# LBM-EPFL/MaD

Hardware: NVIDIA B200
Metric: voxels/sec scale-space+detect+describe(+match) (higher is better)
Workload: dtype f32 grids, f64 line accumulation, u8 x u8 -> s32 matching

## Files before the change

### include/mad_b200.h

```cpp
#ifndef MAD_B200_H
#define MAD_B200_H

#include <stddef.h>
#include <stdint.h>

#ifdef __cplusplus
extern "C" {
#endif

#define MAD_OK 0
#define MAD_ERR_ARG (-1)
#define MAD_ERR_CUDA (-2)
#define MAD_ERR_CAPACITY (-3)
#define MAD_ERR_NODEVICE (-4)

#define MAD_MAX_ORI 36
#define MAD_DSC_LEN 1024

typedef struct MadKeypoint {
    int32_t vox[3];
    int32_t oct;
    float off[3];
    float val;
    int32_t peak[3];
// ... 21 lines not shown
const char* mad_last_error_string(void);
int mad_version(void);
int mad_device_info(int* sm_count, int* cc_major, int* cc_minor);

int mad_publish_small(const void* src_dev, void* dst_host_mapped, int bytes, void* stream);

int mad_copy_to_host(const void* src_dev, void* dst_host_mapped, long long bytes, int n_ctas, void* stream);

long long mad_launch_count(void);
int mad_profile_enable(int on);
int mad_profile_count(void);
int mad_profile_get(int i, const char** name, float* ms);
int mad_profile_reset(void);

int mad_grid_max(const float* grid, long long n, float* out_max_ord, void* stream);
float mad_grid_max_decode(unsigned int ord);
int mad_threshold_normalise(float* grid, long long n, float isovalue, float vmax, int divide, void* stream);
int mad_grid_bbox(const float* grid, int nx, int ny, int nz, int* bbox6, void* stream);
int mad_crop_pad3d(const float* in, int nx, int ny, int nz, int x0, int y0, int z0, int cx, int cy, int cz,
                   int pad, float* out, void* stream);

int mad_pad3d(const float* in, int nx, int ny, int nz, int pad, float* out, void* stream);

size_t mad_upsample_workspace_bytes(int bx, int by, int bz);
int mad_upsample_presmooth(const float* base, int bx, int by, int bz,
                           const double* gauss_w_host, int radius,
                           float* up, void* workspace, size_t workspace_bytes, void* stream);

size_t mad_log_gauss_workspace_bytes(int nx, int ny, int nz);
int mad_log_gauss(const float* grid, int nx, int ny, int nz,
                  const double* w0_host, const double* w2_host, int radius, float scale,
                  float* log_out, float* gauss_out, void* workspace, size_t workspace_bytes,
                  int exact_f64, void* stream);

int mad_gradient(const float* gauss, int nx, int ny, int nz, float* grad4, void* stream);
size_t mad_gradient_tiles(int nx, int ny, int nz);
int mad_gradient_mark(const MadKeypoint* kp, int n_kp, const int* dims_oct_host, int reach_oct0, int reach_oct1,
                      uint8_t* flags_oct0, uint8_t* flags_oct1, void* stream);
int mad_gradient_masked(const float* gauss, int nx, int ny, int nz, float* grad4, uint8_t* flags, void* stream);

int mad_detect(const float* log_grid, int nx, int ny, int nz, int oct, int border,
               float threshold, MadKeypoint* cand, int cap, int* count, void* stream);

size_t mad_sort_keypoints_workspace_bytes(int n);
int mad_sort_keypoints(const MadKeypoint* cand, int n, const int* dims_oct_host,
                       MadKeypoint* out, int* out_count,
                       void* workspace, size_t workspace_bytes, void* stream);

int mad_orient(const float* grad4_oct0, const float* grad4_oct1, const int* dims_oct_host,
               const MadKeypoint* kp, int n_kp, int r, const MadZoneTable* zones112_host,
               const double* r1_table, int lim_main, int lim_sec,
               int32_t* n_ori, int32_t* slots, void* stream);

size_t mad_compact_oriented_workspace_bytes(int n_kp);
int mad_compact_oriented(const int32_t* n_ori, const int32_t* slots, int n_kp,
                         MadOriented* oriented, int cap, int* out_count,
                         void* workspace, size_t workspace_bytes, void* stream);

int mad_describe(const float* grad4_oct0, const float* grad4_oct1, const int* dims_oct_host,
                 const MadKeypoint* kp, const MadOriented* oriented, int n_oriented, int r,
                 const MadZoneTable* zones16_host, const double* rf_table, const double* rf_inv_table,
                 int rf_zones, int16_t* dsc, void* stream);

typedef struct MadDscSet {
    const int16_t* dsc;
    const void* half;
// ... 70 lines not shown
```

### mad_b200/_lib.py

```python
import ctypes as C
import os

import numpy as np

HERE = os.path.dirname(os.path.abspath(__file__))
LIB_PATH = os.path.join(HERE, "libmad_b200.so")


class MadError(RuntimeError):
    pass


if not os.path.exists(LIB_PATH):
    raise ImportError(
        "mad_b200: %s is missing -- build the CUDA library first (python -m mad_b200.build). "
        "There is no CPU fallback." % LIB_PATH)

lib = C.CDLL(LIB_PATH)

KEYPOINT_DTYPE = np.dtype([("vox", "<i4", 3), ("oct", "<i4"), ("off", "<f4", 3), ("val", "<f4"),
                           ("peak", "<i4", 3), ("accepted", "<i4")])
ORIENTED_DTYPE = np.dtype([("kp", "<i4"), ("main", "<i2"), ("sec", "<i2")])
assert KEYPOINT_DTYPE.itemsize == 48 and ORIENTED_DTYPE.itemsize == 8
MAX_ORI = 36
# ... 8 lines not shown


class MadDscSet(C.Structure):
    _fields_ = [("dsc", C.c_void_p), ("half", C.c_void_p), ("norm2", C.c_void_p), ("u8", C.c_void_p),
                ("rnorm", C.c_void_p), ("rows", C.c_int32), ("rows_padded", C.c_int32), ("max_entry", C.c_int32)]


_P = C.c_void_p
_I = C.c_int
_SZ = C.c_size_t

SIGNATURES = {
    "mad_last_error_string": (C.c_char_p, []),
    "mad_version": (_I, []),
    "mad_device_info": (_I, [C.POINTER(_I), C.POINTER(_I), C.POINTER(_I)]),
    "mad_launch_count": (C.c_longlong, []),
    "mad_profile_enable": (_I, [_I]),
    "mad_profile_count": (_I, []),
    "mad_profile_get": (_I, [_I, C.POINTER(C.c_char_p), C.POINTER(C.c_float)]),
    "mad_profile_reset": (_I, []),
    "mad_publish_small": (_I, [_P, _P, _I, _P]),
    "mad_copy_to_host": (_I, [_P, _P, C.c_longlong, _I, _P]),
    "mad_zone_fast_build": (_I, [C.POINTER(MadZoneTable), _P, _P]),
    "mad_grid_max": (_I, [_P, C.c_longlong, _P, _P]),
    "mad_grid_max_decode": (C.c_float, [C.c_uint]),
    "mad_threshold_normalise": (_I, [_P, C.c_longlong, C.c_float, C.c_float, _I, _P]),
    "mad_grid_bbox": (_I, [_P, _I, _I, _I, _P, _P]),
    "mad_crop_pad3d": (_I, [_P, _I, _I, _I, _I, _I, _I, _I, _I, _I, _I, _P, _P]),
    "mad_pad3d": (_I, [_P, _I, _I, _I, _I, _P, _P]),
    "mad_upsample_workspace_bytes": (_SZ, [_I, _I, _I]),
    "mad_upsample_presmooth": (_I, [_P, _I, _I, _I, _P, _I, _P, _P, _SZ, _P]),
    "mad_log_gauss_workspace_bytes": (_SZ, [_I, _I, _I]),
    "mad_log_gauss": (_I, [_P, _I, _I, _I, _P, _P, _I, C.c_float, _P, _P, _P, _SZ, _I, _P]),
    "mad_gradient": (_I, [_P, _I, _I, _I, _P, _P]),
    "mad_gradient_tiles": (_SZ, [_I, _I, _I]),
    "mad_gradient_mark": (_I, [_P, _I, _P, _I, _I, _P, _P, _P]),
    "mad_gradient_masked": (_I, [_P, _I, _I, _I, _P, _P, _P]),
    "mad_detect": (_I, [_P, _I, _I, _I, _I, _I, C.c_float, _P, _I, _P, _P]),
    "mad_sort_keypoints_workspace_bytes": (_SZ, [_I]),
    "mad_sort_keypoints": (_I, [_P, _I, _P, _P, _P, _P, _SZ, _P]),
    "mad_orient": (_I, [_P, _P, _P, _P, _I, _I, C.POINTER(MadZoneTable), _P, _I, _I, _P, _P, _P]),
    "mad_compact_oriented_workspace_bytes": (_SZ, [_I]),
    "mad_compact_oriented": (_I, [_P, _P, _I, _P, _I, _P, _P, _SZ, _P]),
    "mad_describe": (_I, [_P, _P, _P, _P, _P, _I, _I, C.POINTER(MadZoneTable), _P, _P, _I, _P, _P]),
    "mad_dsc_prepare": (_I, [_P, _I, _I, _P, _P, _P, _P, _P]),
    "mad_match_pairs": (_I, [C.POINTER(MadDscSet), C.POINTER(MadDscSet), C.c_double, _P, _P, C.c_uint64, _P, _P]),
    "mad_match_pairs_finish_workspace_bytes": (_SZ, [C.c_longlong]),
    "mad_match_pairs_finish": (_I, [_P, _P, C.c_longlong, _I, _I, _P, _P, _P, _P, _P, _P, _SZ, _P]),
    "mad_match_pairs_finish_dot": (_I, [_P, _P, C.c_longlong, _I, _I, _P, _P, _P, _P, _SZ, _P]),
    "mad_dsc_norms": (_I, [_P, _I, _P, _P]),
    "mad_dsc_to_half": (_I, [_P, _I, _I, _P, _P]),
    "mad_match_segments": (_I, [_I, _I, _I]),
    "mad_match_count": (_I, [C.POINTER(MadDscSet), C.POINTER(MadDscSet), C.c_double, _I, _P, _I, _P]),
    "mad_match_fill": (_I, [C.POINTER(MadDscSet), C.POINTER(MadDscSet), C.c_double, _I, _P, _P, _P, _P, _I, _P]),
    "mad_exclusive_scan_workspace_bytes": (_SZ, [_I]),
    "mad_exclusive_scan_i32_to_i64": (_I, [_P, _I, _P, _P, _P, _SZ, _P]),
    "mad_match_topk_workspace_bytes": (_SZ, [_I, _I, _I, _I]),
    "mad_match_topk": (_I, [C.POINTER(MadDscSet), C.POINTER(MadDscSet), _I, _I, _P, _P, _P, _SZ, _I, _P]),
    "mad_topk_merge": (_I, [_P, _P, _I, _I, _I, _P, _P, _P]),
    "mad_density_splat": (_I, [_P, _P, _I, _P, C.c_double, _I, _I, _I, _I, _P, _P]),
    "mad_normalise_f64": (_I, [_P, C.c_longlong, _P, _P]),
    "mad_conv_full_f64": (_I, [_P, C.c_longlong, _I, C.c_longlong, _P, _I, _P, _I, _P]),
    "mad_mark_used": (_I, [_P, C.c_longlong, _P, _P]),
    "mad_repeatability": (_I, [_P, _P, _P, C.c_longlong, _P, _P, _P, _P, _P, _P, _I, _P, _I, _P, _P, _P, _P, _P,
                               C.c_double, _P, _P]),
    "mad_box_scores_workspace_bytes": (_SZ, [_I, _I, _I]),
# ... 26 lines not shown
```

### mad_b200/csrc/scale_space.cu

```cuda
#include <stdlib.h>
#include <type_traits>

#include "common.cuh"

__global__ void __launch_bounds__(256)
pad3d_kernel(const float* __restrict__ in, int nx, int ny, int nz, int pad, float* __restrict__ out, int ox, int oy, int oz) {
    const int lane = threadIdx.x & 31;
    const long long rows = (long long)ox * oy;
    for (long long row = (long long)blockIdx.x * 8 + (threadIdx.x >> 5); row < rows; row += (long long)gridDim.x * 8) {
        const int x = (int)(row / oy), y = (int)(row - (long long)x * oy);
        const int sx = x - pad, sy = y - pad;
        float* o = out + row * oz;
        if (sx < 0 || sx >= nx || sy < 0 || sy >= ny) {
            for (int z = lane; z < oz; z += 32) o[z] = 0.f;
        } else {
            const float* src = in + ((long long)sx * ny + sy) * nz - pad;
            for (int z = lane; z < oz; z += 32) o[z] = (z >= pad && z < nz + pad) ? __ldg(src + z) : 0.f;
        }
    }
}

extern "C" int mad_pad3d(const float* in, int nx, int ny, int nz, int pad, float* out, void* stream) {
    MAD_CHECK_ARG(in && out && nx > 0 && ny > 0 && nz > 0 && pad >= 0);
    const int ox = nx + 2 * pad, oy = ny + 2 * pad, oz = nz + 2 * pad;
// ... 556 lines not shown
    }
#pragma unroll
    for (int jj = R; jj >= 1; --jj) {
#pragma unroll
        for (int t = 0; t < T; ++t) {
            const ACC s = win[t + R - jj] + win[t + R + jj];
            a0[t] = fma(s, Wt<ACC>::get(w.w0[jj]), a0[t]);
            a2[t] = fma(s, Wt<ACC>::get(w.w2[jj]), a2[t]);
        }
    }
#pragma unroll
    for (int t = 0; t < T; ++t) { o0[t] = (float)a0[t]; o2[t] = (float)a2[t]; }
}

template <int R, int T, typename ACC>
__device__ __forceinline__ void conv_g_rows(const ACC* win, const ConvW& w, float* o0) {
    ACC a0[T];
#pragma unroll
    for (int t = 0; t < T; ++t) a0[t] = win[t + R] * Wt<ACC>::get(w.w0[0]);
#pragma unroll
    for (int jj = R; jj >= 1; --jj) {
#pragma unroll
        for (int t = 0; t < T; ++t) {
            const ACC s = win[t + R - jj] + win[t + R + jj];
            a0[t] = fma(s, Wt<ACC>::get(w.w0[jj]), a0[t]);
        }
    }
#pragma unroll
    for (int t = 0; t < T; ++t) o0[t] = (float)a0[t];
}

__device__ __forceinline__ void cp_async4(float* smem_dst, const float* gsrc) {
    asm volatile("cp.async.ca.shared.global [%0], [%1], 4;" ::"r"((uint32_t)__cvta_generic_to_shared(smem_dst)), "l"(gsrc) : "memory");
}
__device__ __forceinline__ void cp_async_commit() { asm volatile("cp.async.commit_group;" ::: "memory"); }
template <int N>
__device__ __forceinline__ void cp_async_wait() { asm volatile("cp.async.wait_group %0;" ::"n"(N) : "memory"); }

template <int R, typename ACC, int MODE>
__global__ void __launch_bounds__(128)
log_pass_strided_kernel(const float* __restrict__ in0, const float* __restrict__ in1, float* __restrict__ o0,
                        float* __restrict__ o1, float* __restrict__ o2, int n, long long inner,
                        long long total_lines, int seg_len, ConvW w) {
    constexpr int T = ((2 * R) % 8 == 0) ? 8 : 4, W = T + 2 * R;
    constexpr int NA = MODE == 1 ? 2 : 1;
    constexpr int D = 32, PF = D / T - 1;
    constexpr int G0 = 2 * R / T;
    static_assert((2 * R) % T == 0, "window prologue must be whole groups");
    extern __shared__ float ring[];
    const long long g = blockIdx.x * (long long)blockDim.x + threadIdx.x;
    if (g >= total_lines) return;
    const long long o = g / inner, j = g % inner;
    const long long base = o * (long long)n * inner + j;
    const int a0 = blockIdx.y * seg_len;
    const int a1 = min(n, a0 + seg_len);
    const int q_end = a1 - a0 + 2 * R;
    float* my = ring + threadIdx.x;
    auto issue = [&](int grp) {
        const int q0 = grp * T;
        float* dst0 = my + ((q0 & (D - 1)) * NA) * 128;
        const int p0 = a0 - R + q0;
        if (p0 >= 0 && p0 + T <= n && q0 + T <= q_end) {
            const long long off = base + (long long)p0 * inner;
#pragma unroll
            for (int i = 0; i < T; ++i) {
                cp_async4(dst0 + i * NA * 128, in0 + off + (long long)i * inner);
// ... 11 lines not shown
            }
        }
        cp_async_commit();
    };
    static_assert(G0 <= PF + 1, "the initial window must fit the ring");
#pragma unroll
    for (int grp = 0; grp <= PF; ++grp) issue(grp);
    cp_async_wait<PF + 1 - G0>();
    ACC wa[W];
    ACC wb[MODE == 1 ? W : 1];
#pragma unroll
    for (int i = 0; i < 2 * R; ++i) {
        wa[i] = (ACC)my[(i * NA) * 128];
        if (MODE == 1) wb[i] = (ACC)my[(i * NA + 1) * 128];
    }
#pragma unroll
    for (int grp = PF + 1; grp <= PF + G0; ++grp) issue(grp);
    int grp = G0;
    for (int a = a0; a < a1; a += T, ++grp) {
        cp_async_wait<PF>();
#pragma unroll
        for (int i = 0; i < T; ++i) {
            const int slot = (grp * T + i) & (D - 1);
            wa[2 * R + i] = (ACC)my[(slot * NA) * 128];
            if (MODE == 1) wb[2 * R + i] = (ACC)my[(slot * NA + 1) * 128];
        }
        issue(grp + PF + 1);
#pragma unroll
        for (int t = 0; t < T; ++t) {
            if (a + t < a1) {
                const long long off = base + (long long)(a + t) * inner;
                float r0, r2;
                conv_both<R, ACC>(wa, t, w, r0, r2);
                o0[off] = r0;
                o1[off] = r2;
                if (MODE == 1) o2[off] = conv_g<R, ACC>(wb, t, w);
            }
        }
#pragma unroll
        for (int i = 0; i < 2 * R; ++i) {
            wa[i] = wa[i + T];
            if (MODE == 1) wb[i] = wb[i + T];
        }
    }
    cp_async_wait<0>();
}

template <int R, typename ACC>
__global__ void __launch_bounds__(384)
log_pass_z_kernel(const float* __restrict__ P01, const float* __restrict__ Rr, const float* __restrict__ S,
                  float* __restrict__ log_out, float* __restrict__ gauss_out, int nz, long long n_rows,
                  int rows_per_cta, int rs_in, int rs_out, long long n_batches, float scale, ConvW w) {
    constexpr int T = 8, W = T + 2 * R;
    extern __shared__ __align__(16) float zsm[];
    const size_t in_buf = (size_t)3 * rows_per_cta * rs_in;
    float* sout0 = zsm + 2 * in_buf;
    float* sout1 = sout0 + (size_t)rows_per_cta * rs_out;
    const int tid = threadIdx.x;
    const int halo_len = nz + 2 * R;
    auto issue = [&](long long batch, int buf) {
        if (batch < n_batches) {
            const long long row0 = batch * rows_per_cta;
            const int rows = (int)min((long long)rows_per_cta, n_rows - row0);
            float* d0 = zsm + buf * in_buf;
            for (int r = 0; r < rows; ++r) {
                const long long gb = (row0 + r) * nz;
                for (int t = tid; t < halo_len; t += blockDim.x) {
                    const long long src = gb + mad_reflect(t - R, nz);
// ... 48 lines not shown
                if (z0 + t < nz) {
                    sout0[r * rs_out + z0 + t] = m;
                    sout1[r * rs_out + z0 + t] = gs[t];
                }
            }
        }
        __syncthreads();
        for (int r = 0; r < rows; ++r) {
            const long long gb = (row0 + r) * nz;
            for (int t = tid; t < nz; t += blockDim.x) {
                log_out[gb + t] = sout0[r * rs_out + t];
                gauss_out[gb + t] = sout1[r * rs_out + t];
            }
        }
    }
    cp_async_wait<0>();
}

template <int R, int DEPTH = 32>
struct YzCfg {
    static constexpr int T = 8, W = T + 2 * R, D = DEPTH, PF = D / T - 1, G0 = 2 * R / T;
    static constexpr int TZ = 128 - 2 * R;
    static constexpr int CH = 128 / T;
    static constexpr int CW = TZ / CH;
    static constexpr int RS = 128;
    static constexpr int OS = TZ;
    static constexpr size_t ring_bytes = (size_t)D * 2 * 128 * sizeof(float);
    static constexpr size_t stage_bytes = (size_t)3 * T * RS * sizeof(double);
    static constexpr size_t out_bytes = (size_t)2 * T * OS * sizeof(float);
    static constexpr size_t smem = ring_bytes + stage_bytes + out_bytes;
    static constexpr bool ok = TZ % CH == 0 && (CW % 2) == 1 && (2 * R) % T == 0 && G0 <= PF + 1;
};

template <int R, typename ACC, int MINB, int DEPTH>
__global__ void __launch_bounds__(128, MINB)
log_pass_yz_kernel(const float* __restrict__ P0, const float* __restrict__ Q0, float* __restrict__ log_out,
                   float* __restrict__ gauss_out, int ny, int nz, int n_ztiles, float scale, ConvW w) {
    using C = YzCfg<R, DEPTH>;
    static_assert(C::ok, "the fused pass needs a kernel radius that is a multiple of 4");
    constexpr int T = C::T, W = C::W, D = C::D, PF = C::PF, G0 = C::G0, TZ = C::TZ, CH = C::CH, CW = C::CW, RS = C::RS, OS = C::OS;
    constexpr int WB = CW + 2 * R;
    extern __shared__ __align__(16) unsigned char yz_smem[];
    float* ring = reinterpret_cast<float*>(yz_smem);
    double* stage = reinterpret_cast<double*>(yz_smem + C::ring_bytes);
    float* sout = reinterpret_cast<float*>(yz_smem + C::ring_bytes + C::stage_bytes);
    const int tid = threadIdx.x;
    const int x = blockIdx.x / n_ztiles, zt = blockIdx.x - x * n_ztiles;
    const int z0 = zt * TZ;
    int zc = z0 - R + tid;
    if (zc >= nz + R) zc = nz + R - 1;
    zc = mad_reflect(zc, nz);
    const long long plane = (long long)x * ny * nz;
    const long long base = plane + zc;
    const int q_end = ny + 2 * R;
    float* my = ring + tid;
    auto issue = [&](int grp) {
        const int q0 = grp * T;
        float* dst0 = my + ((q0 & (D - 1)) * 2) * 128;
        if (q0 >= R && q0 + T <= ny + R) {
            const float* p0 = P0 + base + (long long)(q0 - R) * nz;
            const float* p1 = Q0 + base + (long long)(q0 - R) * nz;
#pragma unroll
            for (int i = 0; i < T; ++i) {
                cp_async4(dst0 + i * 256, p0 + (long long)i * nz);
                cp_async4(dst0 + i * 256 + 128, p1 + (long long)i * nz);
            }
        } else {
#pragma unroll
            for (int i = 0; i < T; ++i) {
                const int q = q0 + i;
                if (q < q_end) {
                    const long long off = base + (long long)mad_reflect(q - R, ny) * nz;
                    cp_async4(dst0 + i * 256, P0 + off);
                    cp_async4(dst0 + i * 256 + 128, Q0 + off);
                }
            }
        }
        cp_async_commit();
    };
#pragma unroll
    for (int grp = 0; grp <= PF; ++grp) issue(grp);
    cp_async_wait<PF + 1 - G0>();
    ACC wa[W], wb[W];
#pragma unroll
    for (int i = 0; i < 2 * R; ++i) {
        wa[i] = (ACC)my[(i * 2) * 128];
        wb[i] = (ACC)my[(i * 2 + 1) * 128];
    }
#pragma unroll
    for (int grp = PF + 1; grp <= PF + G0; ++grp) issue(grp);
    const int br = tid / CH, bc = tid - br * CH;
    const bool b_active = (z0 + bc * CW) < nz;
    int grp = G0;
    for (int a = 0; a < ny; a += T, ++grp) {
        cp_async_wait<PF>();
#pragma unroll
        for (int i = 0; i < T; ++i) {
            const int slot = (grp * T + i) & (D - 1);
            wa[2 * R + i] = (ACC)my[(slot * 2) * 128];
            wb[2 * R + i] = (ACC)my[(slot * 2 + 1) * 128];
        }
        issue(grp + PF + 1);
        {
            float r0[T], r2[T], r1[T];
            conv_both_rows<R, T, ACC>(wa, w, r0, r2);
            conv_g_rows<R, T, ACC>(wb, w, r1);
#pragma unroll
            for (int t = 0; t < T; ++t) {
                const int slot = t * RS + tid;
                stage[0 * T * RS + slot] = (double)r0[t];
                stage[1 * T * RS + slot] = (double)r2[t];
                stage[2 * T * RS + slot] = (double)r1[t];
            }
        }
#pragma unroll
        for (int i = 0; i < 2 * R; ++i) {
            wa[i] = wa[i + T];
            wb[i] = wb[i + T];
        }
        __syncthreads();
        const int rows = min(T, ny - a);
        if (b_active && br < rows) {
            ACC win[WB];
            auto load_window = [&](int arr) {
                const double* src = stage + (arr * T + br) * RS + bc * CW;
#pragma unroll
                for (int q = 0; q < WB; ++q) win[q] = (ACC)src[q];
            };
            float gs[CW], t3[CW], t2[CW], t1[CW];
            load_window(0);
            conv_both_rows<R, CW, ACC>(win, w, gs, t3);
            load_window(1);
            conv_g_rows<R, CW, ACC>(win, w, t2);
            load_window(2);
            conv_g_rows<R, CW, ACC>(win, w, t1);
#pragma unroll
            for (int t = 0; t < CW; ++t) {
                const float lap = __fadd_rn(__fadd_rn(t1[t], t2[t]), t3[t]);
                float m = __fmul_rn(-lap, scale);
                if (m < 0.f) m = 0.f;
                sout[(0 * T + br) * OS + bc * CW + t] = m;
                sout[(1 * T + br) * OS + bc * CW + t] = gs[t];
            }
        }
        __syncthreads();
        if (tid < TZ && z0 + tid < nz) {
            const float* so = sout + tid;
            float* lo_p = log_out + plane + (long long)a * nz + z0 + tid;
            float* ga_p = gauss_out + plane + (long long)a * nz + z0 + tid;
#pragma unroll
            for (int r = 0; r < T; ++r) {
                if (r < rows) {
                    lo_p[(long long)r * nz] = so[(0 * T + r) * OS];
                    ga_p[(long long)r * nz] = so[(1 * T + r) * OS];
                }
            }
        }
    }
    cp_async_wait<0>();
}

extern "C" size_t mad_log_gauss_workspace_bytes(int nx, int ny, int nz) {
    const size_t v = mad_align_up((size_t)nx * ny * nz * sizeof(float), 256);
    return 5 * v;
}

template <int R, typename ACC>
static int log_gauss_launch(const float* grid, int nx, int ny, int nz, const ConvW& w, float scale, float* log_out,
                            float* gauss_out, float* ws, cudaStream_t st) {
    const size_t v = mad_align_up((size_t)nx * ny * nz * sizeof(float), 256) / sizeof(float);
    float *P0 = ws, *Q0 = ws + v, *P01 = ws + 2 * v, *Rr = ws + 3 * v, *S = ws + 4 * v;
    const int sms = mad_sm_count();
    auto segs_for = [&](long long lines, int n) {
        long long ctas = mad_ceil_div(lines, 128);
        int segs = (int)std::max<long long>(1, std::min<long long>(mad_ceil_div((long long)sms * 8, ctas), mad_ceil_div(n, 64)));
        int seg_len = (int)mad_ceil_div(mad_ceil_div(n, segs), 16) * 16;
        return seg_len;
    };
    {
        const long long inner = (long long)ny * nz;
        const int seg_len = segs_for(inner, nx);
        dim3 grid_dim((unsigned)mad_ceil_div(inner, 128), (unsigned)mad_ceil_div(nx, seg_len));
        MAD_PROF("log_pass_x_kernel", st);
        log_pass_strided_kernel<R, ACC, 0><<<grid_dim, 128, 32 * 1 * 128 * sizeof(float), st>>>(grid, nullptr, P0, Q0, nullptr, nx, inner, inner, seg_len, w);
        MAD_LAUNCH_OK();
    }
    static const bool fused = !(getenv("MAD_LOG_FUSED") && atoi(getenv("MAD_LOG_FUSED")) == 0);
    if constexpr (YzCfg<R>::ok) if (fused) {
        using C = YzCfg<R, 32>;
        const int n_ztiles = (int)mad_ceil_div(nz, C::TZ);
        const unsigned n_cta = (unsigned)((long long)nx * n_ztiles);
        MAD_CUDA(cudaFuncSetAttribute(log_pass_yz_kernel<R, ACC, 3, 32>, cudaFuncAttributeMaxDynamicSharedMemorySize, (int)C::smem));
        MAD_PROF("log_pass_yz_kernel", st);
        log_pass_yz_kernel<R, ACC, 3, 32><<<n_cta, 128, C::smem, st>>>(P0, Q0, log_out, gauss_out, ny, nz, n_ztiles, scale, w);
        MAD_LAUNCH_OK();
        return MAD_OK;
    }
    const long long plane = (long long)ny * nz;
    static const long long slab_env = getenv("MAD_LOG_SLAB") ? atoll(getenv("MAD_LOG_SLAB")) : 0;
    long long slab = slab_env;
    if (slab <= 0 || slab > nx) slab = nx;
    const int n_chunks = (nz + 7) / 8;
    const int rs_in = (n_chunks * 8 + 2 * R + 3) / 4 * 4;
    const int rs_out = (nz + 3) / 4 * 4;
    const size_t row_bytes = (size_t)(2 * 3 * rs_in + 2 * rs_out) * sizeof(float);
    const int max_rows = (int)std::max<size_t>(1, std::min<size_t>(32, (72 * 1024) / row_bytes));
    int rows = 1;
    double best_eff = -1.0;
    for (int r = 1; r <= max_rows; ++r) {
        const long long work = (long long)r * n_chunks;
        const double eff = (double)work / (double)(mad_ceil_div(work, 128) * 128);
        if (eff > best_eff + 1e-9) { best_eff = eff; rows = r; }
    }
    const size_t smem = rows * row_bytes;
    if (smem > 200 * 1024) {
        mad_set_error("mad_log_gauss: z extent %d too long for the shared-memory row stage", nz);
        return MAD_ERR_ARG;
    }
    MAD_CUDA(cudaFuncSetAttribute(log_pass_z_kernel<R, ACC>, cudaFuncAttributeMaxDynamicSharedMemorySize, (int)std::max<size_t>(smem, 48 * 1024)));
    const int ctas_per_sm = (int)std::max<size_t>(1, std::min<size_t>(4, (size_t)(216 * 1024) / std::max<size_t>(smem, 1)));
    for (long long x0 = 0; x0 < nx; x0 += slab) {
        const int sx = (int)std::min<long long>(slab, nx - x0);
        const long long off = x0 * plane;
        {
            const long long inner = nz;
            const long long lines = (long long)sx * nz;
            const int seg_len = segs_for(lines, ny);
            dim3 grid_dim((unsigned)mad_ceil_div(lines, 128), (unsigned)mad_ceil_div(ny, seg_len));
            MAD_PROF("log_pass_y_kernel", st);
            log_pass_strided_kernel<R, ACC, 1><<<grid_dim, 128, 32 * 2 * 128 * sizeof(float), st>>>(P0 + off, Q0 + off, P01, Rr, S, ny, inner, lines, seg_len, w);
            MAD_LAUNCH_OK();
        }
        {
            const long long n_rows = (long long)sx * ny;
            const long long n_batches = mad_ceil_div(n_rows, rows);
            const unsigned grid_z = (unsigned)std::min<long long>(n_batches, (long long)sms * ctas_per_sm);
            MAD_PROF("log_pass_z_kernel", st);
            log_pass_z_kernel<R, ACC><<<grid_z, 128, smem, st>>>(P01, Rr, S, log_out + off, gauss_out + off, nz, n_rows, rows, rs_in, rs_out, n_batches, scale, w);
            MAD_LAUNCH_OK();
        }
    }
    return MAD_OK;
}

extern "C" int mad_log_gauss(const float* grid, int nx, int ny, int nz, const double* w0_host, const double* w2_host,
                             int radius, float scale, float* log_out, float* gauss_out, void* workspace,
                             size_t workspace_bytes, int exact_f64, void* stream) {
    MAD_CHECK_ARG(grid && log_out && gauss_out && workspace && w0_host && w2_host);
    MAD_CHECK_ARG(radius >= 1 && radius <= 16);
    MAD_CHECK_ARG(nx >= 2 * radius + 1 && ny >= 2 * radius + 1 && nz >= 2 * radius + 1);
    MAD_CHECK_ARG(workspace_bytes >= mad_log_gauss_workspace_bytes(nx, ny, nz));
    ConvW w;
    for (int j = 0; j < 17; ++j) w.w0[j] = w.w2[j] = 0.0;
    for (int j = 0; j <= radius; ++j) {
        w.w0[j] = w0_host[radius + j];
        w.w2[j] = w2_host[radius + j];
    }
    float* ws = reinterpret_cast<float*>(workspace);
    cudaStream_t st = (cudaStream_t)stream;
#define MAD_LOG_CASE(RR)                                                                                   \
    case RR:                                                                                               \
        return exact_f64 ? log_gauss_launch<RR, double>(grid, nx, ny, nz, w, scale, log_out, gauss_out, ws, st) \
                         : log_gauss_launch<RR, float>(grid, nx, ny, nz, w, scale, log_out, gauss_out, ws, st);
    switch (radius) {
        MAD_LOG_CASE(4)
        MAD_LOG_CASE(6)
        MAD_LOG_CASE(8)
        MAD_LOG_CASE(10)
        MAD_LOG_CASE(12)
        default:
            mad_set_error("mad_log_gauss: kernel radius %d not instantiated (4, 6, 8, 10, 12)", radius);
            return MAD_ERR_ARG;
    }
#undef MAD_LOG_CASE
}

__device__ __forceinline__ float grad_axis(const float* __restrict__ f, long long c, int i, int n, long long stride) {
    if (i == 0) return __fsub_rn(__ldg(f + c + stride), __ldg(f + c));
    if (i == n - 1) return __fsub_rn(__ldg(f + c), __ldg(f + c - stride));
    return __fmul_rn(__fsub_rn(__ldg(f + c + stride), __ldg(f + c - stride)), 0.5f);
}

constexpr int kGradSlab = 8;
__global__ void __launch_bounds__(256)
gradient_kernel(const float* __restrict__ f, int nx, int ny, int nz, float4* __restrict__ grad) {
    const unsigned plane = (unsigned)ny * (unsigned)nz;
    const unsigned p = blockIdx.x * 256u + threadIdx.x;
    if (p >= plane) return;
    const int y = (int)(p / (unsigned)nz);
    const int z = (int)(p - (unsigned)y * (unsigned)nz);
    const int x0 = blockIdx.y * kGradSlab;
    const int x1 = min(nx, x0 + kGradSlab);
    const long long sx = plane;
    long long c = (long long)x0 * sx + p;
    float prev = (x0 > 0) ? __ldg(f + c - sx) : 0.f;
    float cur = __ldg(f + c);
#pragma unroll 4
    for (int x = x0; x < x1; ++x, c += sx) {
        const float next = (x + 1 < nx) ? __ldg(f + c + sx) : 0.f;
        float4 v;
        if (x == 0) v.x = __fsub_rn(next, cur);
        else if (x == nx - 1) v.x = __fsub_rn(cur, prev);
        else v.x = __fmul_rn(__fsub_rn(next, prev), 0.5f);
        v.y = grad_axis(f, c, y, ny, nz);
        v.z = grad_axis(f, c, z, nz, 1);
        v.w = 0.f;
        grad[c] = v;
// ... 113 lines not shown
```

### mad_b200/pipeline.py

```python
import ctypes as C
import math
import os

import numpy as np
import torch

from . import _lib
from . import tables
from ._lib import call, KEYPOINT_DTYPE, ORIENTED_DTYPE, MAX_ORI, DSC_LEN

def launch_count():
    return int(_lib.lib.mad_launch_count())


def profile_enable(on=True):
    call("mad_profile_reset")
    call("mad_profile_enable", 1 if on else 0)


def profile_records():
    out = []
    name = C.c_char_p()
    ms = C.c_float()
    for i in range(_lib.lib.mad_profile_count()):
# ... 157 lines not shown
    sp.n_input_voxels = nx * ny * nz
    if map_padding:
        bx, by, bz = nx + 2 * map_padding, ny + 2 * map_padding, nz + 2 * map_padding
        base = torch.empty((bx, by, bz), dtype=torch.float32, device=dev)
        call("mad_pad3d", _ptr(grid), nx, ny, nz, int(map_padding), _ptr(base), st)
    else:
        bx, by, bz = nx, ny, nz
        base = grid
    if oct_mode not in ("both", "up", "base"):
        raise _lib.MadError("build_space: oct_mode %r" % (oct_mode,))
    ux, uy, uz = 2 * bx - 1, 2 * by - 1, 2 * bz - 1
    if oct_mode != "base":
        up = torch.empty((ux, uy, uz), dtype=torch.float32, device=dev)
        ws_bytes = _lib.lib.mad_upsample_workspace_bytes(bx, by, bz)
        ws = torch.empty(ws_bytes, dtype=torch.uint8, device=dev)
        if sig_presmooth:
            rad = tables.gaussian_radius(sig_presmooth)
            gw = np.ascontiguousarray(tables.gaussian_weights(sig_presmooth, 0, rad))
            call("mad_upsample_presmooth", _ptr(base), bx, by, bz, _dptr(gw), rad, _ptr(up), _ptr(ws), ws_bytes, st)
        else:
            call("mad_upsample_presmooth", _ptr(base), bx, by, bz, C.c_void_p(0), 0, _ptr(up), _ptr(ws), ws_bytes, st)
        del ws
    if oct_mode == "both":
        sp.grids = [up, base]
        sp.dims = [(ux, uy, uz), (bx, by, bz)]
    else:
        sp.n_oct = 1
        sp.grids = [up] if oct_mode == "up" else [base]
        sp.dims = [(ux, uy, uz) if oct_mode == "up" else (bx, by, bz)]
    rad = tables.gaussian_radius(sig_init)
    w0 = np.ascontiguousarray(tables.gaussian_weights(sig_init, 0, rad))
    w2 = np.ascontiguousarray(tables.gaussian_weights(sig_init, 2, rad))
    scale = float(np.float32(sig_init ** 2))
    for g, (gx, gy, gz) in zip(sp.grids, sp.dims):
        ws_bytes = _lib.lib.mad_log_gauss_workspace_bytes(gx, gy, gz)
        ws = torch.empty(ws_bytes, dtype=torch.uint8, device=dev)
        lg = torch.empty((gx, gy, gz), dtype=torch.float32, device=dev)
        gs = torch.empty((gx, gy, gz), dtype=torch.float32, device=dev)
        call("mad_log_gauss", _ptr(g), gx, gy, gz, _dptr(w0), _dptr(w2), rad, C.c_float(scale), _ptr(lg), _ptr(gs),
             _ptr(ws), ws_bytes, 1 if exact_f64 else 0, st)
        del ws
        gr = torch.empty((gx, gy, gz, 4), dtype=torch.float32, device=dev)
        if full_gradient:
            call("mad_gradient", _ptr(gs), gx, gy, gz, _ptr(gr), st)
            sp.grad_flags.append(None)
        else:
            sp.grad_flags.append(torch.zeros(_lib.lib.mad_gradient_tiles(gx, gy, gz), dtype=torch.uint8, device=dev))
        sp._gauss.append(gs)
        sp.logs.append(lg)
        sp.gauss.append(gs if keep_gauss else None)
        sp.grad4.append(gr)
    if full_gradient and not keep_gauss:
        sp._gauss = []
    if sp.n_oct == 1:
        sp.dims.append((1, 1, 1))
        sp.grad4.append(torch.zeros((1, 1, 1, 4), dtype=torch.float32, device=dev))
        sp.grad_flags.append(None if full_gradient else torch.zeros(1, dtype=torch.uint8, device=dev))
    return sp


class Keypoints(object):

    def __init__(self, table, count):
        self.table = table
        self.count = int(count)
        self._host = None

    def host(self):
        if self._host is None:
            self._host = self.table[:self.count].cpu().numpy().view(KEYPOINT_DTYPE).reshape(-1)
        return self._host

    def __len__(self):
        return self.count
# ... 569 lines not shown
```

Before: 2.255 billion.

## Interleave x-pass outputs as float2 and batch both octaves in one yz launch

The x-pass now writes its two convolution results interleaved as float2, so the fused yz kernel pulls one 8-byte cp.async per row instead of two 4-byte copies from separate arrays. The yz kernel also takes two grid descriptors, so the upsampled and base octaves run in a single launch and their CTAs share the GPU. This is meant to cut launch count, tail underutilisation on the smaller octave, and per-row async copy overhead. In exchange it adds a per-CTA branch to pick the grid, keeps both octave workspaces alive at once (more peak memory), and the plane offsets now use int arithmetic, guarded by new size checks.

```diff
diff --git a/include/mad_b200.h b/include/mad_b200.h
--- a/include/mad_b200.h
+++ b/include/mad_b200.h
@@ -77,6 +77,12 @@
                   const double* w0_host, const double* w2_host, int radius, float scale,
                   float* log_out, float* gauss_out, void* workspace, size_t workspace_bytes,
                   int exact_f64, void* stream);
+int mad_log_gauss_pair(const float* grid0, int nx0, int ny0, int nz0, float* log0, float* gauss0,
+                       void* workspace0, size_t workspace0_bytes,
+                       const float* grid1, int nx1, int ny1, int nz1, float* log1, float* gauss1,
+                       void* workspace1, size_t workspace1_bytes,
+                       const double* w0_host, const double* w2_host, int radius, float scale, int exact_f64,
+                       void* stream);
 
 int mad_gradient(const float* gauss, int nx, int ny, int nz, float* grad4, void* stream);
 size_t mad_gradient_tiles(int nx, int ny, int nz);
diff --git a/mad_b200/_lib.py b/mad_b200/_lib.py
--- a/mad_b200/_lib.py
+++ b/mad_b200/_lib.py
@@ -64,6 +64,8 @@
     "mad_upsample_presmooth": (_I, [_P, _I, _I, _I, _P, _I, _P, _P, _SZ, _P]),
     "mad_log_gauss_workspace_bytes": (_SZ, [_I, _I, _I]),
     "mad_log_gauss": (_I, [_P, _I, _I, _I, _P, _P, _I, C.c_float, _P, _P, _P, _SZ, _I, _P]),
+    "mad_log_gauss_pair": (_I, [_P, _I, _I, _I, _P, _P, _P, _SZ, _P, _I, _I, _I, _P, _P, _P, _SZ,
+                                _P, _P, _I, C.c_float, _I, _P]),
     "mad_gradient": (_I, [_P, _I, _I, _I, _P, _P]),
     "mad_gradient_tiles": (_SZ, [_I, _I, _I]),
     "mad_gradient_mark": (_I, [_P, _I, _P, _I, _I, _P, _P, _P]),
diff --git a/mad_b200/csrc/scale_space.cu b/mad_b200/csrc/scale_space.cu
--- a/mad_b200/csrc/scale_space.cu
+++ b/mad_b200/csrc/scale_space.cu
@@ -612,6 +612,9 @@
 
 __device__ __forceinline__ void cp_async4(float* smem_dst, const float* gsrc) {
     asm volatile("cp.async.ca.shared.global [%0], [%1], 4;" ::"r"((uint32_t)__cvta_generic_to_shared(smem_dst)), "l"(gsrc) : "memory");
+}
+__device__ __forceinline__ void cp_async8(float2* smem_dst, const float2* gsrc) {
+    asm volatile("cp.async.ca.shared.global [%0], [%1], 8;" ::"r"((uint32_t)__cvta_generic_to_shared(smem_dst)), "l"(gsrc) : "memory");
 }
 __device__ __forceinline__ void cp_async_commit() { asm volatile("cp.async.commit_group;" ::: "memory"); }
 template <int N>
@@ -689,8 +692,12 @@
                 const long long off = base + (long long)(a + t) * inner;
                 float r0, r2;
                 conv_both<R, ACC>(wa, t, w, r0, r2);
-                o0[off] = r0;
-                o1[off] = r2;
+                if (MODE == 2) {
+                    reinterpret_cast<float2*>(o0)[off] = make_float2(r0, r2);
+                } else {
+                    o0[off] = r0;
+                    o1[off] = r2;
+                }
                 if (MODE == 1) o2[off] = conv_g<R, ACC>(wb, t, w);
             }
         }
@@ -805,75 +812,88 @@
     static constexpr bool ok = TZ % CH == 0 && (CW % 2) == 1 && (2 * R) % T == 0 && G0 <= PF + 1;
 };
 
+struct YzGrid {
+    const float2* PQ;
+    float* log_out;
+    float* gauss_out;
+    int ny, nz, n_ztiles, ctas;
+};
+
 template <int R, typename ACC, int MINB, int DEPTH>
 __global__ void __launch_bounds__(128, MINB)
-log_pass_yz_kernel(const float* __restrict__ P0, const float* __restrict__ Q0, float* __restrict__ log_out,
-                   float* __restrict__ gauss_out, int ny, int nz, int n_ztiles, float scale, ConvW w) {
+log_pass_yz_kernel(YzGrid g0, YzGrid g1, float scale, ConvW w) {
     using C = YzCfg<R, DEPTH>;
     static_assert(C::ok, "the fused pass needs a kernel radius that is a multiple of 4");
-    constexpr int T = C::T, W = C::W, D = C::D, PF = C::PF, G0 = C::G0, TZ = C::TZ, CH = C::CH, CW = C::CW, RS = C::RS, OS = C::OS;
+    constexpr int T = C::T, W = C::W, D = C::D, PF = C::PF, G0 = C::G0, TZ = C::TZ, CH = C::CH, CW = C::CW,
+                  RS = C::RS, OS = C::OS;
     constexpr int WB = CW + 2 * R;
     extern __shared__ __align__(16) unsigned char yz_smem[];
-    float* ring = reinterpret_cast<float*>(yz_smem);
+    float2* ring = reinterpret_cast<float2*>(yz_smem);
     double* stage = reinterpret_cast<double*>(yz_smem + C::ring_bytes);
     float* sout = reinterpret_cast<float*>(yz_smem + C::ring_bytes + C::stage_bytes);
     const int tid = threadIdx.x;
-    const int x = blockIdx.x / n_ztiles, zt = blockIdx.x - x * n_ztiles;
+    const bool second = (int)blockIdx.x >= g0.ctas;
+    const int b = (int)blockIdx.x - (second ? g0.ctas : 0);
+    const int ny = second ? g1.ny : g0.ny, nz = second ? g1.nz : g0.nz;
+    const int n_ztiles = second ? g1.n_ztiles : g0.n_ztiles;
+    const int x = b / n_ztiles, zt = b - x * n_ztiles;
     const int z0 = zt * TZ;
+    const size_t plane = (size_t)x * ny * nz;
+    const float2* PQ = (second ? g1.PQ : g0.PQ) + plane;
+    float* log_out = (second ? g1.log_out : g0.log_out) + plane;
+    float* gauss_out = (second ? g1.gauss_out : g0.gauss_out) + plane;
     int zc = z0 - R + tid;
     if (zc >= nz + R) zc = nz + R - 1;
     zc = mad_reflect(zc, nz);
-    const long long plane = (long long)x * ny * nz;
-    const long long base = plane + zc;
     const int q_end = ny + 2 * R;
-    float* my = ring + tid;
-    auto issue = [&](int grp) {
-        const int q0 = grp * T;
-        float* dst0 = my + ((q0 & (D - 1)) * 2) * 128;
+    float2* my = ring + tid;
+    int q0 = 0;
+    const float2* p_row = PQ + zc - (long long)R * nz;
+    auto issue = [&]() {
+        float2* dst0 = my + (q0 & (D - 1)) * 128;
         if (q0 >= R && q0 + T <= ny + R) {
-            const float* p0 = P0 + base + (long long)(q0 - R) * nz;
-            const float* p1 = Q0 + base + (long long)(q0 - R) * nz;
+            const float2* p = p_row;
 #pragma unroll
             for (int i = 0; i < T; ++i) {
-                cp_async4(dst0 + i * 256, p0 + (long long)i * nz);
-                cp_async4(dst0 + i * 256 + 128, p1 + (long long)i * nz);
+                cp_async8(dst0 + i * 128, p);
+                p += nz;
             }
         } else {
 #pragma unroll
             for (int i = 0; i < T; ++i) {
-                const int q = q0 + i;
-                if (q < q_end) {
-                    const long long off = base + (long long)mad_reflect(q - R, ny) * nz;
-                    cp_async4(dst0 + i * 256, P0 + off);
-                    cp_async4(dst0 + i * 256 + 128, Q0 + off);
-                }
+                if (q0 + i < q_end)
+                    cp_async8(dst0 + i * 128, p_row + (long long)(mad_reflect(q0 + i - R, ny) - (q0 - R)) * nz);
             }
         }
         cp_async_commit();
+        q0 += T;
+        p_row += T * nz;
     };
 #pragma unroll
-    for (int grp = 0; grp <= PF; ++grp) issue(grp);
+    for (int grp = 0; grp <= PF; ++grp) issue();
     cp_async_wait<PF + 1 - G0>();
     ACC wa[W], wb[W];
 #pragma unroll
     for (int i = 0; i < 2 * R; ++i) {
-        wa[i] = (ACC)my[(i * 2) * 128];
-        wb[i] = (ACC)my[(i * 2 + 1) * 128];
-    }
-#pragma unroll
-    for (int grp = PF + 1; grp <= PF + G0; ++grp) issue(grp);
+        const float2 v = my[i * 128];
+        wa[i] = (ACC)v.x;
+        wb[i] = (ACC)v.y;
+    }
+#pragma unroll
+    for (int grp = PF + 1; grp <= PF + G0; ++grp) issue();
     const int br = tid / CH, bc = tid - br * CH;
     const bool b_active = (z0 + bc * CW) < nz;
     int grp = G0;
     for (int a = 0; a < ny; a += T, ++grp) {
         cp_async_wait<PF>();
+        const float2* src = my + ((grp * T) & (D - 1)) * 128;
 #pragma unroll
         for (int i = 0; i < T; ++i) {
-            const int slot = (grp * T + i) & (D - 1);
-            wa[2 * R + i] = (ACC)my[(slot * 2) * 128];
-            wb[2 * R + i] = (ACC)my[(slot * 2 + 1) * 128];
-        }
-        issue(grp + PF + 1);
+            const float2 v = src[i * 128];
+            wa[2 * R + i] = (ACC)v.x;
+            wb[2 * R + i] = (ACC)v.y;
+        }
+        issue();
         {
             float r0[T], r2[T], r1[T];
             conv_both_rows<R, T, ACC>(wa, w, r0, r2);
@@ -896,9 +916,9 @@
         if (b_active && br < rows) {
             ACC win[WB];
             auto load_window = [&](int arr) {
-                const double* src = stage + (arr * T + br) * RS + bc * CW;
-#pragma unroll
-                for (int q = 0; q < WB; ++q) win[q] = (ACC)src[q];
+                const double* s = stage + (arr * T + br) * RS + bc * CW;
+#pragma unroll
+                for (int q = 0; q < WB; ++q) win[q] = (ACC)s[q];
             };
             float gs[CW], t3[CW], t2[CW], t1[CW];
             load_window(0);
@@ -919,14 +939,16 @@
         __syncthreads();
         if (tid < TZ && z0 + tid < nz) {
             const float* so = sout + tid;
-            float* lo_p = log_out + plane + (long long)a * nz + z0 + tid;
-            float* ga_p = gauss_out + plane + (long long)a * nz + z0 + tid;
+            float* lo = log_out + (a * nz + z0 + tid);
+            float* ga = gauss_out + (a * nz + z0 + tid);
 #pragma unroll
             for (int r = 0; r < T; ++r) {
                 if (r < rows) {
-                    lo_p[(long long)r * nz] = so[(0 * T + r) * OS];
-                    ga_p[(long long)r * nz] = so[(1 * T + r) * OS];
+                    *lo = so[(0 * T + r) * OS];
+                    *ga = so[(1 * T + r) * OS];
                 }
+                lo += nz;
+                ga += nz;
             }
         }
     }
@@ -938,11 +960,20 @@
     return 5 * v;
 }
 
+struct LogGrid {
+    const float* grid;
+    int nx, ny, nz;
+    float* log_out;
+    float* gauss_out;
+    float* ws;
+};
+
 template <int R, typename ACC>
-static int log_gauss_launch(const float* grid, int nx, int ny, int nz, const ConvW& w, float scale, float* log_out,
-                            float* gauss_out, float* ws, cudaStream_t st) {
-    const size_t v = mad_align_up((size_t)nx * ny * nz * sizeof(float), 256) / sizeof(float);
-    float *P0 = ws, *Q0 = ws + v, *P01 = ws + 2 * v, *Rr = ws + 3 * v, *S = ws + 4 * v;
+static int log_gauss_launch(const LogGrid* grids, int n_grids, const ConvW& w, float scale, cudaStream_t st) {
+    auto parts = [](const LogGrid& g, int i) {
+        const size_t v = mad_align_up((size_t)g.nx * g.ny * g.nz * sizeof(float), 256) / sizeof(float);
+        return g.ws + i * v;
+    };
     const int sms = mad_sm_count();
     auto segs_for = [&](long long lines, int n) {
         long long ctas = mad_ceil_div(lines, 128);
@@ -950,91 +981,113 @@
         int seg_len = (int)mad_ceil_div(mad_ceil_div(n, segs), 16) * 16;
         return seg_len;
     };
-    {
-        const long long inner = (long long)ny * nz;
-        const int seg_len = segs_for(inner, nx);
-        dim3 grid_dim((unsigned)mad_ceil_div(inner, 128), (unsigned)mad_ceil_div(nx, seg_len));
+    static const bool fused_env = !(getenv("MAD_LOG_FUSED") && atoi(getenv("MAD_LOG_FUSED")) == 0);
+    const bool fused = YzCfg<R>::ok && fused_env;
+    for (int i = 0; i < n_grids; ++i) {
+        const LogGrid& g = grids[i];
+        const long long inner = (long long)g.ny * g.nz;
+        const int seg_len = segs_for(inner, g.nx);
+        dim3 grid_dim((unsigned)mad_ceil_div(inner, 128), (unsigned)mad_ceil_div(g.nx, seg_len));
         MAD_PROF("log_pass_x_kernel", st);
-        log_pass_strided_kernel<R, ACC, 0><<<grid_dim, 128, 32 * 1 * 128 * sizeof(float), st>>>(grid, nullptr, P0, Q0, nullptr, nx, inner, inner, seg_len, w);
+        if (fused)
+            log_pass_strided_kernel<R, ACC, 2><<<grid_dim, 128, 32 * 1 * 128 * sizeof(float), st>>>(
+                g.grid, nullptr, parts(g, 0), nullptr, nullptr, g.nx, inner, inner, seg_len, w);
+        else
+            log_pass_strided_kernel<R, ACC, 0><<<grid_dim, 128, 32 * 1 * 128 * sizeof(float), st>>>(
+                g.grid, nullptr, parts(g, 0), parts(g, 1), nullptr, g.nx, inner, inner, seg_len, w);
         MAD_LAUNCH_OK();
     }
-    static const bool fused = !(getenv("MAD_LOG_FUSED") && atoi(getenv("MAD_LOG_FUSED")) == 0);
     if constexpr (YzCfg<R>::ok) if (fused) {
         using C = YzCfg<R, 32>;
-        const int n_ztiles = (int)mad_ceil_div(nz, C::TZ);
-        const unsigned n_cta = (unsigned)((long long)nx * n_ztiles);
+        YzGrid yz[2];
+        for (int i = 0; i < n_grids; ++i) {
+            const LogGrid& g = grids[i];
+            const int n_ztiles = (int)mad_ceil_div(g.nz, C::TZ);
+            yz[i] = YzGrid{reinterpret_cast<const float2*>(parts(g, 0)), g.log_out, g.gauss_out, g.ny, g.nz, n_ztiles, g.nx * n_ztiles};
+        }
+        if (n_grids == 1) yz[1] = yz[0];
+        const unsigned n_cta = (unsigned)((long long)yz[0].ctas + (n_grids == 2 ? yz[1].ctas : 0));
         MAD_CUDA(cudaFuncSetAttribute(log_pass_yz_kernel<R, ACC, 3, 32>, cudaFuncAttributeMaxDynamicSharedMemorySize, (int)C::smem));
         MAD_PROF("log_pass_yz_kernel", st);
-        log_pass_yz_kernel<R, ACC, 3, 32><<<n_cta, 128, C::smem, st>>>(P0, Q0, log_out, gauss_out, ny, nz, n_ztiles, scale, w);
+        log_pass_yz_kernel<R, ACC, 3, 32><<<n_cta, 128, C::smem, st>>>(yz[0], yz[1], scale, w);
         MAD_LAUNCH_OK();
         return MAD_OK;
     }
-    const long long plane = (long long)ny * nz;
-    static const long long slab_env = getenv("MAD_LOG_SLAB") ? atoll(getenv("MAD_LOG_SLAB")) : 0;
-    long long slab = slab_env;
-    if (slab <= 0 || slab > nx) slab = nx;
-    const int n_chunks = (nz + 7) / 8;
-    const int rs_in = (n_chunks * 8 + 2 * R + 3) / 4 * 4;
-    const int rs_out = (nz + 3) / 4 * 4;
-    const size_t row_bytes = (size_t)(2 * 3 * rs_in + 2 * rs_out) * sizeof(float);
-    const int max_rows = (int)std::max<size_t>(1, std::min<size_t>(32, (72 * 1024) / row_bytes));
-    int rows = 1;
-    double best_eff = -1.0;
-    for (int r = 1; r <= max_rows; ++r) {
-        const long long work = (long long)r * n_chunks;
-        const double eff = (double)work / (double)(mad_ceil_div(work, 128) * 128);
-        if (eff > best_eff + 1e-9) { best_eff = eff; rows = r; }
-    }
-    const size_t smem = rows * row_bytes;
-    if (smem > 200 * 1024) {
-        mad_set_error("mad_log_gauss: z extent %d too long for the shared-memory row stage", nz);
-        return MAD_ERR_ARG;
-    }
-    MAD_CUDA(cudaFuncSetAttribute(log_pass_z_kernel<R, ACC>, cudaFuncAttributeMaxDynamicSharedMemorySize, (int)std::max<size_t>(smem, 48 * 1024)));
-    const int ctas_per_sm = (int)std::max<size_t>(1, std::min<size_t>(4, (size_t)(216 * 1024) / std::max<size_t>(smem, 1)));
-    for (long long x0 = 0; x0 < nx; x0 += slab) {
-        const int sx = (int)std::min<long long>(slab, nx - x0);
-        const long long off = x0 * plane;
-        {
-            const long long inner = nz;
-            const long long lines = (long long)sx * nz;
-            const int seg_len = segs_for(lines, ny);
-            dim3 grid_dim((unsigned)mad_ceil_div(lines, 128), (unsigned)mad_ceil_div(ny, seg_len));
-            MAD_PROF("log_pass_y_kernel", st);
-            log_pass_strided_kernel<R, ACC, 1><<<grid_dim, 128, 32 * 2 * 128 * sizeof(float), st>>>(P0 + off, Q0 + off, P01, Rr, S, ny, inner, lines, seg_len, w);
-            MAD_LAUNCH_OK();
-        }
-        {
-            const long long n_rows = (long long)sx * ny;
-            const long long n_batches = mad_ceil_div(n_rows, rows);
-            const unsigned grid_z = (unsigned)std::min<long long>(n_batches, (long long)sms * ctas_per_sm);
-            MAD_PROF("log_pass_z_kernel", st);
-            log_pass_z_kernel<R, ACC><<<grid_z, 128, smem, st>>>(P01, Rr, S, log_out + off, gauss_out + off, nz, n_rows, rows, rs_in, rs_out, n_batches, scale, w);
-            MAD_LAUNCH_OK();
+    for (int i = 0; i < n_grids; ++i) {
+        const int nx = grids[i].nx, ny = grids[i].ny, nz = grids[i].nz;
+        const float *P0 = parts(grids[i], 0), *Q0 = parts(grids[i], 1);
+        float *P01 = parts(grids[i], 2), *Rr = parts(grids[i], 3), *S = parts(grids[i], 4);
+        float *log_out = grids[i].log_out, *gauss_out = grids[i].gauss_out;
+        const long long plane = (long long)ny * nz;
+        static const long long slab_env = getenv("MAD_LOG_SLAB") ? atoll(getenv("MAD_LOG_SLAB")) : 0;
+        long long slab = slab_env;
+        if (slab <= 0 || slab > nx) slab = nx;
+        const int n_chunks = (nz + 7) / 8;
+        const int rs_in = (n_chunks * 8 + 2 * R + 3) / 4 * 4;
+        const int rs_out = (nz + 3) / 4 * 4;
+        const size_t row_bytes = (size_t)(2 * 3 * rs_in + 2 * rs_out) * sizeof(float);
+        const int max_rows = (int)std::max<size_t>(1, std::min<size_t>(32, (72 * 1024) / row_bytes));
+        int rows = 1;
+        double best_eff = -1.0;
+        for (int r = 1; r <= max_rows; ++r) {
+            const long long work = (long long)r * n_chunks;
+            const double eff = (double)work / (double)(mad_ceil_div(work, 128) * 128);
+            if (eff > best_eff + 1e-9) { best_eff = eff; rows = r; }
+        }
+        const size_t smem = rows * row_bytes;
+        if (smem > 200 * 1024) {
+            mad_set_error("mad_log_gauss: z extent %d too long for the shared-memory row stage", nz);
+            return MAD_ERR_ARG;
+        }
+        MAD_CUDA(cudaFuncSetAttribute(log_pass_z_kernel<R, ACC>, cudaFuncAttributeMaxDynamicSharedMemorySize, (int)std::max<size_t>(smem, 48 * 1024)));
+        const int ctas_per_sm = (int)std::max<size_t>(1, std::min<size_t>(4, (size_t)(216 * 1024) / std::max<size_t>(smem, 1)));
+        for (long long x0 = 0; x0 < nx; x0 += slab) {
+            const int sx = (int)std::min<long long>(slab, nx - x0);
+            const long long off = x0 * plane;
+            {
+                const long long inner = nz;
+                const long long lines = (long long)sx * nz;
+                const int seg_len = segs_for(lines, ny);
+                dim3 grid_dim((unsigned)mad_ceil_div(lines, 128), (unsigned)mad_ceil_div(ny, seg_len));
+                MAD_PROF("log_pass_y_kernel", st);
+                log_pass_strided_kernel<R, ACC, 1><<<grid_dim, 128, 32 * 2 * 128 * sizeof(float), st>>>(P0 + off, Q0 + off, P01, Rr, S, ny, inner, lines, seg_len, w);
+                MAD_LAUNCH_OK();
+            }
+            {
+                const long long n_rows = (long long)sx * ny;
+                const long long n_batches = mad_ceil_div(n_rows, rows);
+                const unsigned grid_z = (unsigned)std::min<long long>(n_batches, (long long)sms * ctas_per_sm);
+                MAD_PROF("log_pass_z_kernel", st);
+                log_pass_z_kernel<R, ACC><<<grid_z, 128, smem, st>>>(P01, Rr, S, log_out + off, gauss_out + off, nz, n_rows, rows, rs_in, rs_out, n_batches, scale, w);
+                MAD_LAUNCH_OK();
+            }
         }
     }
     return MAD_OK;
 }
 
-extern "C" int mad_log_gauss(const float* grid, int nx, int ny, int nz, const double* w0_host, const double* w2_host,
-                             int radius, float scale, float* log_out, float* gauss_out, void* workspace,
-                             size_t workspace_bytes, int exact_f64, void* stream) {
-    MAD_CHECK_ARG(grid && log_out && gauss_out && workspace && w0_host && w2_host);
+static int log_gauss_run(const LogGrid* grids, int n_grids, size_t* ws_bytes, const double* w0_host, const double* w2_host,
+                         int radius, float scale, int exact_f64, cudaStream_t st) {
+    MAD_CHECK_ARG(w0_host && w2_host);
     MAD_CHECK_ARG(radius >= 1 && radius <= 16);
-    MAD_CHECK_ARG(nx >= 2 * radius + 1 && ny >= 2 * radius + 1 && nz >= 2 * radius + 1);
-    MAD_CHECK_ARG(workspace_bytes >= mad_log_gauss_workspace_bytes(nx, ny, nz));
+    for (int i = 0; i < n_grids; ++i) {
+        const LogGrid& g = grids[i];
+        MAD_CHECK_ARG(g.grid && g.log_out && g.gauss_out && g.ws);
+        MAD_CHECK_ARG(g.nx >= 2 * radius + 1 && g.ny >= 2 * radius + 1 && g.nz >= 2 * radius + 1);
+        MAD_CHECK_ARG(ws_bytes[i] >= mad_log_gauss_workspace_bytes(g.nx, g.ny, g.nz));
+        MAD_CHECK_ARG((long long)(g.ny + 128) * g.nz < 0x7fffffffLL);
+        MAD_CHECK_ARG((long long)g.nx * mad_ceil_div(g.nz, 8) < 0x3fffffffLL);
+    }
     ConvW w;
     for (int j = 0; j < 17; ++j) w.w0[j] = w.w2[j] = 0.0;
     for (int j = 0; j <= radius; ++j) {
         w.w0[j] = w0_host[radius + j];
         w.w2[j] = w2_host[radius + j];
     }
-    float* ws = reinterpret_cast<float*>(workspace);
-    cudaStream_t st = (cudaStream_t)stream;
-#define MAD_LOG_CASE(RR)                                                                                   \
-    case RR:                                                                                               \
-        return exact_f64 ? log_gauss_launch<RR, double>(grid, nx, ny, nz, w, scale, log_out, gauss_out, ws, st) \
-                         : log_gauss_launch<RR, float>(grid, nx, ny, nz, w, scale, log_out, gauss_out, ws, st);
+#define MAD_LOG_CASE(RR)                                                                          \
+    case RR:                                                                                      \
+        return exact_f64 ? log_gauss_launch<RR, double>(grids, n_grids, w, scale, st)             \
+                         : log_gauss_launch<RR, float>(grids, n_grids, w, scale, st);
     switch (radius) {
         MAD_LOG_CASE(4)
         MAD_LOG_CASE(6)
@@ -1046,6 +1099,25 @@
             return MAD_ERR_ARG;
     }
 #undef MAD_LOG_CASE
+}
+
+extern "C" int mad_log_gauss(const float* grid, int nx, int ny, int nz, const double* w0_host, const double* w2_host,
+                             int radius, float scale, float* log_out, float* gauss_out, void* workspace,
+                             size_t workspace_bytes, int exact_f64, void* stream) {
+    const LogGrid g{grid, nx, ny, nz, log_out, gauss_out, reinterpret_cast<float*>(workspace)};
+    return log_gauss_run(&g, 1, &workspace_bytes, w0_host, w2_host, radius, scale, exact_f64, (cudaStream_t)stream);
+}
+
+extern "C" int mad_log_gauss_pair(const float* grid0, int nx0, int ny0, int nz0, float* log0, float* gauss0,
+                                  void* workspace0, size_t workspace0_bytes,
+                                  const float* grid1, int nx1, int ny1, int nz1, float* log1, float* gauss1,
+                                  void* workspace1, size_t workspace1_bytes,
+                                  const double* w0_host, const double* w2_host, int radius, float scale, int exact_f64,
+                                  void* stream) {
+    const LogGrid g[2] = {{grid0, nx0, ny0, nz0, log0, gauss0, reinterpret_cast<float*>(workspace0)},
+                          {grid1, nx1, ny1, nz1, log1, gauss1, reinterpret_cast<float*>(workspace1)}};
+    size_t ws_bytes[2] = {workspace0_bytes, workspace1_bytes};
+    return log_gauss_run(g, 2, ws_bytes, w0_host, w2_host, radius, scale, exact_f64, (cudaStream_t)stream);
 }
 
 __device__ __forceinline__ float grad_axis(const float* __restrict__ f, long long c, int i, int n, long long stride) {
diff --git a/mad_b200/pipeline.py b/mad_b200/pipeline.py
--- a/mad_b200/pipeline.py
+++ b/mad_b200/pipeline.py
@@ -213,14 +213,21 @@
     w0 = np.ascontiguousarray(tables.gaussian_weights(sig_init, 0, rad))
     w2 = np.ascontiguousarray(tables.gaussian_weights(sig_init, 2, rad))
     scale = float(np.float32(sig_init ** 2))
-    for g, (gx, gy, gz) in zip(sp.grids, sp.dims):
-        ws_bytes = _lib.lib.mad_log_gauss_workspace_bytes(gx, gy, gz)
-        ws = torch.empty(ws_bytes, dtype=torch.uint8, device=dev)
-        lg = torch.empty((gx, gy, gz), dtype=torch.float32, device=dev)
-        gs = torch.empty((gx, gy, gz), dtype=torch.float32, device=dev)
-        call("mad_log_gauss", _ptr(g), gx, gy, gz, _dptr(w0), _dptr(w2), rad, C.c_float(scale), _ptr(lg), _ptr(gs),
-             _ptr(ws), ws_bytes, 1 if exact_f64 else 0, st)
-        del ws
+    ws_bytes = [_lib.lib.mad_log_gauss_workspace_bytes(gx, gy, gz) for gx, gy, gz in sp.dims]
+    ws = [torch.empty(b, dtype=torch.uint8, device=dev) for b in ws_bytes]
+    lgs = [torch.empty(d, dtype=torch.float32, device=dev) for d in sp.dims]
+    gss = [torch.empty(d, dtype=torch.float32, device=dev) for d in sp.dims]
+    if len(sp.grids) == 2:
+        args = []
+        for g, (gx, gy, gz), lg, gs, w, b in zip(sp.grids, sp.dims, lgs, gss, ws, ws_bytes):
+            args += [_ptr(g), gx, gy, gz, _ptr(lg), _ptr(gs), _ptr(w), b]
+        call("mad_log_gauss_pair", *args, _dptr(w0), _dptr(w2), rad, C.c_float(scale), 1 if exact_f64 else 0, st)
+    else:
+        (gx, gy, gz), = sp.dims
+        call("mad_log_gauss", _ptr(sp.grids[0]), gx, gy, gz, _dptr(w0), _dptr(w2), rad, C.c_float(scale), _ptr(lgs[0]),
+             _ptr(gss[0]), _ptr(ws[0]), ws_bytes[0], 1 if exact_f64 else 0, st)
+    del ws
+    for (gx, gy, gz), lg, gs in zip(sp.dims, lgs, gss):
         gr = torch.empty((gx, gy, gz, 4), dtype=torch.float32, device=dev)
         if full_gradient:
             call("mad_gradient", _ptr(gs), gx, gy, gz, _ptr(gr), st)
```

New measurement: 2.337 billion, median of 6. 1.04x the previous value.
